# TinyMPC/TinyMPC

Measured on AMD Instinct MI355X. Metric: QP solves/sec (+ ADMM iters/sec), 64k-batch quadrotor hover, higher is better.
Workload: dtype f64; 1 GPU; quadrotor_hovering (nx=12, nu=4, N=10), 65536 identical instances per GPU, closed-loop MPC steps from a cold start (BASELINE configs[1]); batch_per_gpu=65536, total_batch=65536, parallelism=batch-sharded x1, mpc_steps_per_launch=8, stats_exchange=none (one rank), launcher=plain process

## Files before the change

### tinympc_amd/csrc/admm_kernel.hip.h

```cpp
#pragma once
#include <hip/hip_runtime.h>
#include <stdint.h>

namespace tinympc_amd {

enum : int {
    VEC_CB = 0,
    VEC_CF = 1,
    VEC_QR = 2,
    VEC_SMASK = 3,
    VEC_NIM = 4,
    VEC_SOCFLAG = 5,
    VEC_CONE_BASE = 6,
    VEC_CONE_MU = 7,
    VEC_RHO = 8,
    VEC_LINFLAG = 9,
    VEC_TLINFLAG = 10,
    VEC_COUNT = 16,
};
struct LaneTab {
    int cols, lw;
    constexpr int MB() const { return 0; }
    constexpr int MF1() const { return cols * lw; }
    constexpr int MF2() const { return 2 * cols * lw; }
// ... 40 lines not shown
    double* dbg_pd;
    uint2* accum;
    int* iter_log;
    double* u0_log;
    double rho, tol_pri, tol_dua;
    int batch, max_iter, check_termination;
    int steps;
    const double* traj;
    const int* traj_offsets;
    int traj_points, traj_step0;
    int reset_duals;
    const double* het_tabs;
    double *lslack, *ldual, *tlslack, *tldual;
    int n_lin, n_tlin;
    int cold, store_mask;
    const int* index;
    const int* count;
    int iter_base;
    int* next_index;
    int* next_count;
    double *arho, *aK, *aP, *aC1, *aC2;
    const double* atab;
    double arho_min, arho_max;
    int aclip;
    int ref_shared;
    int* work_counter;
    int reverse;
    const int* perm;
    int perm_count;
    double* vz_stream;
    int pf_mask, pf_shards, pf_static;
    unsigned* pf_counter;
    unsigned pf_base[8];
};

#define DPP_FMA(acc, src, m, lane, bank) "v_fmac_f64_dpp %[" acc "], %[" src "], %[" m "] row_newbcast:" lane " row_mask:0xf bank_mask:" bank "\n\t"
#define DPP_REP1(S) S(0, 0)
#define DPP_REP2(S) DPP_REP1(S) S(1, 1)
#define DPP_REP3(S) DPP_REP2(S) S(2, 0)
#define DPP_REP4(S) DPP_REP3(S) S(3, 1)
#define DPP_REP5(S) DPP_REP4(S) S(4, 0)
#define DPP_REP6(S) DPP_REP5(S) S(5, 1)
#define DPP_REP7(S) DPP_REP6(S) S(6, 0)
#define DPP_REP8(S) DPP_REP7(S) S(7, 1)
#define DPP_REP9(S) DPP_REP8(S) S(8, 0)
#define DPP_REP10(S) DPP_REP9(S) S(9, 1)
#define DPP_REP11(S) DPP_REP10(S) S(10, 0)
#define DPP_REP12(S) DPP_REP11(S) S(11, 1)
#define DPP_REP13(S) DPP_REP12(S) S(12, 0)
#define DPP_REP14(S) DPP_REP13(S) S(13, 1)
#define DPP_REP15(S) DPP_REP14(S) S(14, 0)
#define DPP_REP16(S) DPP_REP15(S) S(15, 1)
#define DPP_REP_(K, S) DPP_REP##K(S)
#define DPP_REP(K, S) DPP_REP_(K, S)
#define DPP_ROW_M(k, p) , [m##k] "v"(m[k])
#define DPP_ROW_A(k, p) , [a##k] "v"(ma[k])
#define DPP_ROW_B(k, p) , [b##k] "v"(mb_[k])
#define RING2_COL(k, p) DPP_FMA("a" #p, "src", "m" #k, "%[c0]+" #k, "0xf")
#define RING1_COL(k, p) DPP_FMA("a0", "src", "m" #k, "%[c0]+" #k, "0xf")
#define RING_CASE(K)                                                                                                                     \
    if constexpr (NCOL == K)                                                                                                             \
        asm("s_nop 1\n\t" DPP_REP(K, RING2_COL) : [a0] "+&v"(a0), [a1] "+&v"(a1) : [src] "v"(src), [c0] "i"(COL0) DPP_REP(K, DPP_ROW_M));
#define RING1_CASE(K)                                                                                                                    \
    if constexpr (NCOL == K)                                                                                                             \
        asm("s_nop 1\n\t" DPP_REP(K, RING1_COL) : [a0] "+&v"(a0) : [src] "v"(src), [c0] "i"(COL0) DPP_REP(K, DPP_ROW_M));

// ... 183 lines not shown
    if constexpr (fused_shape(NA, NB)) {
        double vm;
        asm("v_add_f64 %[tt], %[xi], %[g]\n\t"
            "v_max_f64 %[vm], %[lo], %[tt]\n\t"
            DPP_REP(TINYMPC_FUSED_NX, HFWD_COL_A_LO)
            "v_min_f64 %[vn], %[hi], %[vm]\n\t"
            DPP_REP(TINYMPC_FUSED_NX, HFWD_COL_A_HI)
            "v_mov_b64 %[xn], %[t]\n\t"
            "v_add_f64 %[gnew], %[tt], -%[vn]\n\t"
            DPP_REP(TINYMPC_FUSED_NU, HFWD_COL_B_LO)
            "s_nop 0\n\t"
            DPP_REP(TINYMPC_FUSED_NU, HFWD_COL_B_HI)
            : [tt] "=&v"(tt), [vm] "=&v"(vm), [vn] "=&v"(vn), [xn] "=&v"(xn), [t] "+&v"(t), [gnew] "=&v"(gnew)
            : [xi] "v"(xi), [g] "v"(g), [lo] "v"(lo), [hi] "v"(hi), FUSED_ROW_OPERANDS);
    }
#endif
}

__device__ __forceinline__ double vmax64(double a, double b) {
    double r;
    asm("v_max_f64 %0, %1, %2" : "=v"(r) : "v"(a), "v"(b));
    return r;
}
__device__ __forceinline__ double vmin64(double a, double b) {
    double r;
    asm("v_min_f64 %0, %1, %2" : "=v"(r) : "v"(a), "v"(b));
    return r;
}
__device__ __forceinline__ double pinned_sub64(double a, double b) {
    double r = a - b;
    asm volatile("" : "+v"(r));
    return r;
}
__device__ __forceinline__ double vclamp64(double lo, double hi, double t) {
    double r;
    asm("v_max_f64 %0, %1, %2\n\tv_min_f64 %0, %3, %0" : "=&v"(r) : "v"(lo), "v"(t), "v"(hi));
    return r;
}

__device__ __forceinline__ double vmax_abs64(double a, double b) {
    double r;
    asm("v_max_f64 %0, %1, |%2|" : "=v"(r) : "v"(a), "v"(b));
    return r;
}
template <bool OPAQUE>
__device__ __forceinline__ double resid_max(double a, double b) {
    if constexpr (OPAQUE) return vmax_abs64(a, b);
    else return fmax(a, fabs(b));
}

#ifndef TINYMPC_PRIM_STORE
#define TINYMPC_PRIM_STORE 1
#endif
#ifndef TINYMPC_REF_LOAD
#define TINYMPC_REF_LOAD 1
#endif
#ifndef TINYMPC_FULL_LINE_STORES
#define TINYMPC_FULL_LINE_STORES 2
#endif
__device__ __forceinline__ double load_ref(const double* p) {
#if TINYMPC_REF_LOAD == 1
    return __builtin_nontemporal_load(p);
#else
    return *p;
#endif
}
// ... 92 lines not shown
#pragma clang fp contract(off)
    for (int c = S0 + t; c < n; c += LPI_) {
        const int at = (inst * n + c) * csl + R0;
        const double* tk = tab + c * tab_stride;
        double z[NF], t0[NF];
#pragma unroll
        for (int r = 0; r < NF; ++r) { z[r] = pv[at + r]; t0[r] = z[r]; }
        for (int k = 0; k < nk; ++k) {
            double cv = 0.0;
#pragma unroll
            for (int r = 0; r < NF; ++r) { const double pr = tk[k * LW_ + R0 + r] * z[r]; cv = cv + pr; }
            const double bk = tk[KMAX_ * LW_ + k * LW_ + R0];
            if (cv > bk) {
                const double dist = (cv - bk) / tk[2 * KMAX_ * LW_ + k * LW_ + R0];
#pragma unroll
                for (int r = 0; r < NF; ++r) { const double pr = dist * tk[k * LW_ + R0 + r]; z[r] = z[r] - pr; }
            }
        }
#pragma unroll
        for (int r = 0; r < NF; ++r) { pv[at + r] = z[r]; pg[at + r] = t0[r] - z[r]; }
    }
}

template <int NX, int NU, int N, bool SOC, bool DBG, int MODE, int LIN = 0, bool HET = false, int KMAX = LIN_KMAX, bool ADAPT = false, bool UB = false, bool HALF = false,
          bool PF = false>
__global__ __launch_bounds__(64)
__attribute__((amdgpu_waves_per_eu(LIN != 0 ? solve_kernel_lin_waves(NX, NU, N, SOC, LIN, KMAX, UB) : solve_kernel_waves_per_simd(NX + NU, N, SOC, false, ADAPT),
                                   LIN != 0 ? solve_kernel_lin_waves(NX, NU, N, SOC, LIN, KMAX, UB) : solve_kernel_waves_per_simd(NX + NU, N, SOC, false, ADAPT))))
void admm_solve_kernel(const SolveArgs P) {
    constexpr bool LS = (LIN & 1) != 0, LT = (LIN & 2) != 0;
    constexpr int NZ = NX + NU;
    static_assert(NZ <= 16, "one instance per 16-lane DPP row");
    constexpr bool FUSED = MODE == 2 && LIN == 0 && fused_shape(NX, NU);
    static_assert(!HALF || (NZ <= 8 && FUSED && !SOC && !DBG && !HET && !ADAPT), "half rows: nx+nu <= 8, the plain box kernel on its fused step blocks");
    static_assert(!PF || (MODE == 2 && !SOC && !DBG && LIN == 0 && !HET && !ADAPT), "prefetch form: the plain box kernel");
    constexpr int RL = HALF ? 8 : 16;
    constexpr int IPW = 64 / RL;
    constexpr int RECD = N * NZ;
    constexpr int PF_PIECES = (IPW * RECD * 8 + 1023) / 1024;
    constexpr int PF_ARR = PF_PIECES * 128;
    constexpr unsigned long long RMASK = HALF ? 0xFFull : 0xFFFFull;
    const int lane = threadIdx.x & 63;
    const int j = lane & (RL - 1);
    const int grp = lane / RL;
    const bool is_state = j < NX;
    const bool is_input = (j >= NX) && (j < NZ);

    __shared__ double sPt[NX * 16];
    __shared__ double sLo[UB ? 1 : N * 16];
    __shared__ double sHi[UB ? 1 : N * 16];
    __shared__ double sLin[LS ? 3 * KMAX * 16 : 1];
    __shared__ double sTLin[LT ? 3 * N * KMAX * 16 : 1];
#ifndef TINYMPC_SOC_PD
#define TINYMPC_SOC_PD 2
#endif
    constexpr int SPD = TINYMPC_SOC_PD, SPR = SPD + 1;
    constexpr int CS = SOC ? ((NZ + 1) | 1) : 1;
    constexpr int SLOT_D = 3 * CS;
    constexpr int PL_GC = CS, PL_VC = 2 * CS;
    __shared__ double sC[SOC ? (4 * N + 1) * SLOT_D : 1];
    __shared__ double sP[ADAPT ? 4 * NX * NX : 1];
    constexpr int AKC = NX > NU ? NX : NU;
    constexpr bool HA = HET && ADAPT;
    __shared__ double sTab[(ADAPT && !HET) ? 3 * 16 * AKC : 1];
    __shared__ double sDl[ADAPT ? 4 * ADAPT_LOG : 1];
    if constexpr (ADAPT && !HET)
        for (int e = lane; e < 3 * 16 * AKC; e += 64) {
            const int t = e / (16 * AKC), r = e % (16 * AKC);
            sTab[e] = P.atab[t * 256 + (r % AKC) * 16 + r / AKC];
        }
    if constexpr (LS) for (int e = lane; e < 3 * KMAX * 16; e += 64) sLin[e] = P.tab[TAB_BOUNDS + 2 * N * 16 + e];
    if constexpr (LT) for (int e = lane; e < 3 * N * KMAX * 16; e += 64) sTLin[e] = P.tab[TAB_BOUNDS + 2 * N * 16 + 3 * KMAX * 16 + e];
    for (int e = lane; e < NX * 16; e += 64) sPt[e] = P.tab[TAB_PT + e];
    for (int e = lane; e < N * 16; e += 64) {
        if constexpr (!UB) {
            sLo[e] = P.tab[TAB_BOUNDS + e];
            sHi[e] = P.tab[TAB_BOUNDS + N * 16 + e];
        }
    }
    double mb[NZ], mf1[NX], mf2[NU];
#pragma unroll
    for (int k = 0; k < NZ; ++k) mb[k] = P.tab[TAB_MB + k * 16 + j];
#pragma unroll
    for (int k = 0; k < NX; ++k) mf1[k] = P.tab[TAB_MF1 + k * 16 + j];
#pragma unroll
    for (int k = 0; k < NU; ++k) mf2[k] = P.tab[TAB_MF2 + (NX + k) * 16 + j];
    double cb = P.tab[TAB_VEC + VEC_CB * 16 + j];
    double cf = P.tab[TAB_VEC + VEC_CF * 16 + j];
    double qr = P.tab[TAB_VEC + VEC_QR * 16 + j];
    const double smask = P.tab[TAB_VEC + VEC_SMASK * 16 + j];
    const double nim = P.tab[TAB_VEC + VEC_NIM * 16 + j];
    bool soc_lane = false, proj_lane = false;
    int cone_base = -1, cone_c = 0;
    double socmask = 0.0;
    if constexpr (SOC) {
        socmask = P.tab[TAB_VEC + VEC_SOCFLAG * 16 + j];
        soc_lane = socmask != 0.0;
        cone_base = (int)P.tab[TAB_VEC + VEC_CONE_BASE * 16 + j];
// ... 17 lines not shown
            int t = p * 16 + j;
            item_at[p] = 4 * N * SLOT_D; item_mu[p] = 1.0f;
            if (heads && p * 16 < soc_items_of(heads, NX, N)) soc_passes = p + 1;
            for (unsigned m = heads; m; m &= m - 1) {
                const int hb = __builtin_ctz(m);
                const int cnt = hb < NX ? N : N - 1;
                if (t >= 0 && t < cnt) {
                    item_at[p] = (grp * N + t + (hb < NX ? 0 : 1)) * SLOT_D + hb;
                    item_mu[p] = (float)P.tab[TAB_VEC + VEC_CONE_MU * 16 + hb];
                    t = -1;
                } else if (t >= 0) t -= cnt;
            }
            item_rmu[p] = 1.0f / item_mu[p];
            const unsigned mb_ = __float_as_uint(item_mu[p]);
            const bool p2 = (mb_ & 0x807FFFFFu) == 0u && (mb_ >> 23) >= 127u - 60u && (mb_ >> 23) <= 127u + 60u;
            if (__builtin_amdgcn_ballot_w64(!p2) != 0ull) mu_pow2 = false;
        }
    }
    bool lin_lane = false, tlin_lane = false;
    if constexpr (LS) lin_lane = P.tab[TAB_VEC + VEC_LINFLAG * 16 + j] != 0.0;
    if constexpr (LT) tlin_lane = P.tab[TAB_VEC + VEC_TLINFLAG * 16 + j] != 0.0;
    constexpr bool LPL = solve_kernel_lin_planes(NX, NU, N, SOC, LIN, KMAX, UB);
    constexpr bool LSP = LS && LPL, LTP = LT && LPL, LSR = LS && !LPL, LTR = LT && !LPL;
    constexpr int CSL = LPL ? ((NZ + 1) | 1) : 1;
    __shared__ double sLV[LSP ? 4 * N * CSL : 1], sLG[LSP ? 4 * N * CSL : 1];
    __shared__ double sTV[LTP ? 4 * N * CSL : 1], sTG[LTP ? 4 * N * CSL : 1];
    double ones[(LSR || LTR) ? 16 : 1];
#pragma unroll
    for (int k = 0; k < ((LSR || LTR) ? 16 : 1); ++k) ones[k] = 1.0;
    bool lin_x_on = false, lin_u_on = false, tlin_x_on = false, tlin_u_on = false;
    if constexpr (LS) { lin_x_on = P.tab[TAB_VEC + VEC_LINFLAG * 16] != 0.0; lin_u_on = P.tab[TAB_VEC + VEC_LINFLAG * 16 + NX] != 0.0; }
    if constexpr (LT) { tlin_x_on = P.tab[TAB_VEC + VEC_TLINFLAG * 16] != 0.0; tlin_u_on = P.tab[TAB_VEC + VEC_TLINFLAG * 16 + NX] != 0.0; }
    double rho = P.rho;
    __builtin_amdgcn_fence(__ATOMIC_RELEASE, "wavefront");
    __builtin_amdgcn_wave_barrier();

    const double lo_u = P.tab[TAB_BOUNDS + (N > 1 ? 16 : 0) + j], hi_u = P.tab[TAB_BOUNDS + N * 16 + (N > 1 ? 16 : 0) + j];
    const double lo_u0 = P.tab[TAB_BOUNDS + j], hi_u0 = P.tab[TAB_BOUNDS + N * 16 + j];
    const int ninst = PF ? P.batch : (P.index ? *P.count : (P.perm ? P.perm_count : P.batch));
    const int ntiles = (ninst + IPW - 1) / IPW;
    const bool resumed = !PF && P.index != nullptr;
    const bool has_traj = !PF && P.traj != nullptr;
    extern __shared__ __attribute__((aligned(16))) double sPF[];
    typedef const __attribute__((address_space(1))) void* pf_gptr;
    typedef __attribute__((address_space(3))) void* pf_lptr;
    constexpr int PF_S0 = 128, PF_S1 = PF_S0 + PF_ARR, PF_S2 = PF_S1 + PF_ARR, PF_S3 = PF_S2 + PF_ARR;
    auto pf_issue = [&](const int t) {
        const int tl = P.reverse ? ntiles - 1 - t : t;
        __builtin_amdgcn_global_load_lds((pf_gptr)(P.x0 + ((size_t)tl * (IPW * NX) + (size_t)lane * 2)), (pf_lptr)sPF, 16, 0, 0);
        const size_t t0 = (size_t)tl * (IPW * RECD) + (size_t)lane * 2;
        auto arr = [&](const double* p, const int at) {
#pragma unroll
            for (int q = 0; q < PF_PIECES; ++q) __builtin_amdgcn_global_load_lds((pf_gptr)(p + t0 + q * 128), (pf_lptr)(sPF + at + q * 128), 16, 0, 0);
        };
        if (!P.cold) { arr(P.slack, PF_S0); arr(P.dual, PF_S1); arr(P.slack_prev, PF_S2); }
        if (P.pf_mask & 8) arr(P.ref, P.cold ? PF_S0 : PF_S3);
    };
    unsigned pf_ticket = 0u;
    const int pf_shard = PF ? (int)(blockIdx.x % (unsigned)(P.pf_shards > 0 ? P.pf_shards : 1)) : 0;
    typedef __attribute__((address_space(1))) unsigned* pf_ctr_t;
    unsigned long long pf_ctr_bits = PF ? (unsigned long long)(P.pf_counter + 16 * pf_shard) : 0ull;
    if constexpr (PF) asm volatile("" : "+v"(pf_ctr_bits));
    const pf_ctr_t pf_ctr = (pf_ctr_t)pf_ctr_bits;
    auto pf_draw = [&]() { return lane == 0 ? __hip_atomic_fetch_add(pf_ctr, 1u, __ATOMIC_RELAXED, __HIP_MEMORY_SCOPE_AGENT) : 0u; };
    const unsigned pf_base = PF ? P.pf_base[pf_shard] : 0u;
    int pf_next = 0, pf_i = 0;
// ... 135 lines not shown
                    VP[s] = warm ? pfVP[s] : 0.0;
                    QX[s] = pfQXs[s];
                    X[s] = 0.0;
                    if (s == N - 1) ref_last = pf_rl;
                    continue;
                }
                const double r = valid ? (P.ref_shared ? P.ref[off - (size_t)b * (N * NZ)] : load_ref(P.ref + off)) : 0.0;
                VN[s] = warm ? P.slack[off] : 0.0;
                G[s] = warm ? P.dual[off] : 0.0;
                VP[s] = warm ? P.slack_prev[off] : 0.0;
                QX[s] = -(r * qr);
                X[s] = 0.0;
                if (s == N - 1) ref_last = r;
                if constexpr (SOC) {
                    double vc0 = (warm && soc_lane) ? (resumed ? P.cslack : P.prim)[off] : 0.0;
                    const double gc0 = (warm && soc_lane) ? P.cdual[off] : 0.0;
                    if (s == 0 && is_state && soc_lane && !resumed) vc0 = x0v_in;
                    sC[cw + s * SLOT_D] = vc0 - gc0;
                    sC[cw + s * SLOT_D + PL_GC] = gc0;
                    sC[cw + s * SLOT_D + PL_VC] = vc0;
                }
                if constexpr (LS) {
                    const double vl0 = (warm && lin_lane) ? (resumed ? P.lslack : P.prim)[off] : 0.0;
                    const double gl0 = (warm && lin_lane) ? P.ldual[off] : 0.0;
                    if constexpr (LSP) { sLV[cl + s * CSL] = vl0; sLG[cl + s * CSL] = gl0; } else { VL[s] = vl0; GL[s] = gl0; }
                }
                if constexpr (LT) {
                    const double vt0 = (warm && tlin_lane) ? (resumed ? P.tlslack : P.prim)[off] : 0.0;
                    const double gt0 = (warm && tlin_lane) ? P.tldual[off] : 0.0;
                    if constexpr (LTP) { sTV[cl + s * CSL] = vt0; sTG[cl + s * CSL] = gt0; } else { VT[s] = vt0; GT[s] = gt0; }
                }
                if constexpr (DBG) { Qd[s] = 0.0; Pd[s] = 0.0; Dd[s] = 0.0; }
            }
            double x0v = x0v_in;
            auto terminal_term = [&]() {
                double pt[NX];
#pragma unroll
                for (int k = 0; k < NX; ++k)
                    pt[k] = ADAPT ? sP[grp * NX * NX + k + NX * (is_state ? j : 0)] : (HET ? het[TAB_PT + k * 16 + j] : sPt[k * 16 + j]);
                double xp = 0.0;
                if constexpr (HALF) ring1_half<0, NX>(xp, ref_last, pt);
                else xp = ring_sum<MODE, 0, NX>(0.0, ref_last, pt);
                qx_last_plain = QX[N - 1];
                QX[N - 1] = is_state ? -xp : QX[N - 1];
            };
            int ndl = 0;
            auto flush_c = [&](int n) {
                __builtin_amdgcn_fence(__ATOMIC_RELEASE, "wavefront");
                __builtin_amdgcn_wave_barrier();
                if (P.aC2 && is_state) {
                    double* c2 = P.aC2 + (size_t)b * (NX * NX) + NX * j;
                    double v[NX], d[NX];
#pragma unroll
                    for (int k = 0; k < NX; ++k) { v[k] = c2[k]; d[k] = P.atab[(HA ? (size_t)b * ATAB_DOUBLES : (size_t)0) + ATAB_DC2 + k * 16 + j]; }
                    for (int i = 0; i < n; ++i) {
                        const double dl = sDl[grp * ADAPT_LOG + i];
#pragma unroll
                        for (int k = 0; k < NX; ++k) v[k] = taylor_step(v[k], dl, d[k]);
                    }
#pragma unroll
                    for (int k = 0; k < NX; ++k) c2[k] = v[k];
                }
                if (P.aC1 && j < NU) {
                    double* c1 = P.aC1 + (size_t)b * (NU * NU) + NU * j;
                    double v[NU], d[NU];
#pragma unroll
// ... 95 lines not shown
                            if constexpr (LT) ql = fma(-rho, tlin_w(N - 1), ql);
                            Qd[N - 1] = is_state ? ql : t;
                            Pd[N - 1] = t;
                        }
                    }
                    double pcur = qhi;
                    if constexpr (HALF) {
                        double tmpv = VN[N - 2] - G[N - 2];
#pragma unroll
                        for (int i = N - 2; i >= 0; --i) {
                            double qlo, res, dnp, tmpn;
                            constexpr int dummy = 0;
                            const int in = i > 0 ? i - 1 : dummy;
                            fused_backward_step_half<NX, NU>(qlo, res, dnp, tmpn, tmpv, VN[in], G[in], QX[i], rho, smask, cb, nim, cf, pcur, qhi, mb, mb + NX);
                            if (i + 1 <= N - 2) Dn[i + 1] = dnp;
                            tmpv = tmpn;
                            pcur = res;
                            qhi = qlo;
                        }
                        Dn[0] = fma(pcur, nim, cf);
                    }
#pragma unroll
                    for (int i = N - 2; i >= 0 && !HALF; --i) {
                        if constexpr (SOC) {
                            if (i >= SPD) wr[(i - SPD) % SPR] = sC[cw + (i - SPD) * SLOT_D];
                        }
                        if constexpr (LSP) { if (i >= SPD) { lvr[(i - SPD) % SPR] = sLV[cl + (i - SPD) * CSL]; lgr[(i - SPD) % SPR] = sLG[cl + (i - SPD) * CSL]; } }
                        if constexpr (LTP) { if (i >= SPD) { tvr[(i - SPD) % SPR] = sTV[cl + (i - SPD) * CSL]; tgr[(i - SPD) % SPR] = sTG[cl + (i - SPD) * CSL]; } }
                        if constexpr (SOC || LPL) __builtin_amdgcn_sched_barrier(0);
                        if constexpr (FUSED) {
                            double qlo, res;
                            if constexpr (SOC) fused_backward_step_soc<NX, NU>(qlo, res, VN[i], G[i], QX[i], wr[i % SPR], rho, smask, cb, pcur, qhi, mb, mb + NX);
                            else fused_backward_step<NX, NU>(qlo, res, VN[i], G[i], QX[i], rho, smask, cb, pcur, qhi, mb, mb + NX);
                            pcur = res;
                            Dn[i] = fma(res, nim, cf);
                            if constexpr (DBG) { Qd[i] = qlo; Pd[i] = res; Dd[i + 1] = res; }
                            qhi = qlo;
                            continue;
                        }
                        double qlo = fma(-rho, VN[i] - G[i], QX[i]);
                        if constexpr (SOC) qlo = fma(-rho, wr[i % SPR], qlo);
                        if constexpr (LS) qlo = fma(-rho, lin_w(i), qlo);
                        if constexpr (LT) qlo = fma(-rho, tlin_w(i), qlo);
                        const double res = ring_sum2<MODE, NX, NU>(fma(qlo, smask, cb), pcur, mb, qhi, mb + NX);
                        pcur = res;
                        Dn[i] = fma(res, nim, cf);
                        if constexpr (DBG) { Qd[i] = qlo; Pd[i] = res; Dd[i + 1] = res; }
                        qhi = qlo;
                    }
                    constexpr bool LAZY_RES = N <= 12;
                    constexpr bool TIGHT = FUSED && !HALF && LAZY_RES && !SOC && NX % 4 == 0;
                    double pmax = 0.0, dmax = 0.0;
                    auto slot_update = [&](const int s, const double lo, const double hi, const double gcv, const double glv, const double gtv) {
                        const double xi = X[s];
                        const double t = xi + G[s];
                        const double vn = TIGHT ? vclamp64(lo, hi, t) : vmin64(hi, vmax64(lo, t));
                        if constexpr (!LAZY_RES) {
                            pmax = resid_max<true>(pmax, xi - vn);
                            dmax = resid_max<true>(dmax, VP[s] - vn);
                        }
                        G[s] = t - vn;
                        VN[s] = vn;
                        if constexpr (SOC) {
                            sC[cw + s * SLOT_D] = fma(xi, socmask, gcv);
                        }
                        if constexpr (LSP) sLV[cl + s * CSL] = (lin_lane && (is_state || s >= 1)) ? (xi + glv) : 0.0;
                        if constexpr (LTP) sTV[cl + s * CSL] = (tlin_lane && (is_state || s >= 1)) ? (xi + gtv) : 0.0;
                        if constexpr (LSR || LTR) {
                            auto halfspaces = [&](double z, const double* tabk, const int nk) {
                                for (int k = 0; k < nk; ++k) {
                                    const double a = tabk[k * 16 + j];
                                    const double bk = tabk[KMAX * 16 + k * 16 + j];
                                    const double nn = tabk[2 * KMAX * 16 + k * 16 + j];
                                    const double prod = a * z;
                                    double cs = 0.0, ci = 0.0;
                                    ring1<0, NX>(cs, prod, ones);
                                    ring1<NX, NU>(ci, prod, ones);
                                    const double cv = is_state ? cs : ci;
                                    if (cv > bk) {
#pragma clang fp contract(off)
                                        const double pr = ((cv - bk) / nn) * a;
                                        z = z - pr;
                                    }
                                }
// ... 66 lines not shown
                                tt_d = tt; vn_d = vn;
                            } else G[i] = tt - vn;
                            VN[i] = vn;
                            if constexpr (SOC) sC[cw + i * SLOT_D] = fma(xi, socmask, gr[i % SPR]);
                            lo_c = lo_n; hi_c = hi_n;
                            continue;
                        }
                        const double t = ring_sum<MODE, 0, NX>(Dn[i], X[i], mf1);
                        X[i + 1] = ring_short<MODE, NX, NU>(t, t, mf2);
                        slot_update(i, lo_c, hi_c, gr[SOC ? i % SPR : 0], glr[LSP ? i % SPR : 0], gtr[LTP ? i % SPR : 0]);
                        lo_c = lo_n; hi_c = hi_n;
                    }
                    if constexpr (TIGHT && N >= 2) G[N - 2] = tt_d - vn_d;
                    (void)tt_d; (void)vn_d;
                    slot_update(N - 1, lo_c, hi_c, gr[SOC ? (N - 1) % SPR : 0], glr[LSP ? (N - 1) % SPR : 0], gtr[LTP ? (N - 1) % SPR : 0]);
                    if constexpr (LPL) {
                        __builtin_amdgcn_fence(__ATOMIC_RELEASE, "wavefront");
                        __builtin_amdgcn_wave_barrier();
                        if constexpr (LSP) {
                            if (lin_x_on) project_halfspace_columns<NX, KMAX, 16, 16>(j, grp, N, CSL, 0, 0, sLV, sLG, sLin, 0, P.n_lin);
                            if (lin_u_on) project_halfspace_columns<NU, KMAX, 16, 16>(j, grp, N, CSL, NX, 1, sLV, sLG, sLin, 0, P.n_lin);
                        }
                        if constexpr (LTP) {
                            if (tlin_x_on) project_halfspace_columns<NX, KMAX, 16, 16>(j, grp, N, CSL, 0, 0, sTV, sTG, sTLin, 3 * KMAX * 16, P.n_tlin);
                            if (tlin_u_on) project_halfspace_columns<NU, KMAX, 16, 16>(j, grp, N, CSL, NX, 1, sTV, sTG, sTLin, 3 * KMAX * 16, P.n_tlin);
                        }
                        __builtin_amdgcn_fence(__ATOMIC_RELEASE, "wavefront");
                        __builtin_amdgcn_wave_barrier();
                    }
                    bool conv = false;
                    auto termination = [&]() {
                        if (countdown > 0 && --countdown == 0) {
                            countdown = P.check_termination;
                            checked = 1;
                            constexpr int PS0 = N >= 2 ? 1 : 0, PS1 = N - 1;
                            auto lost = [&](const int s) {
                                return (int)(fabs(X[s] - VN[s]) >= P.tol_pri) | (int)(fabs(VP[s] - VN[s]) * rho >= P.tol_dua);
                            };
                            const bool maybe = ((int)!(rho > 0.0) | (int)!(lost(PS0) | lost(PS1))) != 0;
                            unsigned long long fold = __ballot(maybe);
                            fold &= fold >> 1; fold &= fold >> 2; fold &= fold >> 4;
                            if constexpr (!HALF) fold &= fold >> 8;
                            const bool any_row = (fold & (HALF ? 0x0101010101010101ull : 0x0001000100010001ull)) != 0ull;
                            const bool last_test = (P.max_iter - 1 - it) < P.check_termination;
                            if (last_test || any_row) {
                                if constexpr (LAZY_RES) {
#pragma unroll
                                    for (int s = 0; s < N; ++s) {
                                        pmax = resid_max<false>(pmax, X[s] - VN[s]);
                                        dmax = resid_max<false>(dmax, VP[s] - VN[s]);
                                    }
                                }
                                rp = pmax;
                                rd = dmax * rho;
                                const bool ok = (rp < P.tol_pri) && (rd < P.tol_dua);
                                const unsigned long long bal = __ballot(ok);
                                conv = ((bal >> (grp * RL)) & RMASK) == RMASK;
                            }
                        }
                    };
                    if constexpr (SOC) {
                        __builtin_amdgcn_fence(__ATOMIC_RELEASE, "wavefront");
                        __builtin_amdgcn_wave_barrier();
                        double n0 = sC[item_at[0]], n1 = sC[item_at[0] + 1], n2 = sC[item_at[0] + 2];
#pragma unroll
                        for (int d = 1; d <= SPR && d <= N; ++d) wr[(N - d) % SPR] = sC[cw + (N - d) * SLOT_D];
                        termination();
                        bool any_exact = false;
#pragma unroll
                        for (int p = 0; p < SOC_PASSES; ++p) {
                            if (p > 0 && p >= soc_passes) break;
                            const int at = item_at[p];
                            if (p > 0) { n0 = sC[at]; n1 = sC[at + 1]; n2 = sC[at + 2]; }
                            const double s0 = n0, s1 = n1, s2 = n2;
                            if (soc_all_inside(s0, s1, s2, item_mu[p])) {
                                sC[at + PL_VC] = s0; sC[at + PL_VC + 1] = s1; sC[at + PL_VC + 2] = s2;
                                if (!gcz[p]) {
                                    sC[at + PL_GC] = 0.0; sC[at + PL_GC + 1] = 0.0; sC[at + PL_GC + 2] = 0.0;
                                    gcz[p] = true;
                                }
                            } else {
                                double r0, r1, r2;
                                soc_project3(s0, s1, s2, item_mu[p], item_rmu[p], mu_pow2, r0, r1, r2);
                                const double g0 = s0 - r0, g1 = s1 - r1, g2 = s2 - r2;
                                sC[at + PL_VC] = r0; sC[at + PL_VC + 1] = r1; sC[at + PL_VC + 2] = r2;
                                sC[at + PL_GC] = g0; sC[at + PL_GC + 1] = g1; sC[at + PL_GC + 2] = g2;
                                sC[at] = r0 - g0; sC[at + 1] = r1 - g1; sC[at + 2] = r2 - g2;
                                gcz[p] = false;
                                any_exact = true;
                            }
                        }
                        if (it == iter0 && !proj_lane) {
#pragma unroll
                            for (int s = 0; s < N; ++s) sC[cw + s * SLOT_D + PL_GC] = 0.0;
                        }
                        __builtin_amdgcn_fence(__ATOMIC_RELEASE, "wavefront");
                        __builtin_amdgcn_wave_barrier();
                        if (any_exact) {
#pragma unroll
                            for (int d = 1; d <= SPR && d <= N; ++d) wr[(N - d) % SPR] = sC[cw + (N - d) * SLOT_D];
                        }
                    }
                    iter += 1;
                    if constexpr (ADAPT) {
                        if (it > 0 && it % 5 == 0) {
                            double at[NX];
#pragma unroll
                            for (int k = 0; k < NX; ++k) at[k] = HA ? atab_i[ATAB_AT + k * 16 + j] : sTab[j * AKC + k];
                            double pri_res = 0.0, ax_max = 0.0, z_max = 0.0, dual_res = 0.0, px_max = 0.0, aty_max = 0.0, q_max = 0.0;
                            double pxq_max = 0.0;
#pragma unroll
                            for (int i = 0; i < N - 1; ++i) {
                                const double axs = ring_sum<MODE, 0, NX>(0.0, X[i], mf1);
                                const double dyn = ring_short<MODE, NX, NU>(axs, is_input ? X[i + 1] : 0.0, mf2) - X[i + 1];
                                const double a = is_state ? dyn : X[i + 1];
                                const double zz = VN[i + 1];
                                const bool on = is_state || is_input;
                                pri_res = fmax(pri_res, on ? fabs(a - zz) : 0.0);
                                ax_max = fmax(ax_max, on ? fabs(a) : 0.0);
                                z_max = fmax(z_max, on ? fabs(zz) : 0.0);
                                const double init = is_state ? (i >= 1 ? -G[i] : 0.0) : G[i + 1];
                                const double aty = ring_sum<MODE, 0, NX>(init, G[i + 1], at);
                                const double xs = is_state ? X[i] : X[i + 1];
                                const double px = qr * xs;
                                dual_res = fmax(dual_res, on ? fabs((px + px) + aty) : 0.0);
                                pxq_max = fmax(pxq_max, on ? fabs(px) : 0.0);
                                aty_max = fmax(aty_max, on ? fabs(aty) : 0.0);
                            }
                            {
                                double prow[NX];
#pragma unroll
                                for (int k = 0; k < NX; ++k) prow[k] = sP[grp * NX * NX + (is_state ? j : 0) + NX * k];
                                const double pxl = ring_sum<MODE, 0, NX>(0.0, X[N - 1], prow);
                                const double ql = qr * X[N - 1];
                                const double atyl = -G[N - 1];
                                dual_res = fmax(dual_res, is_state ? fabs((pxl + ql) + atyl) : 0.0);
// ... 6 lines not shown
                            const double pri_norm = fmax(ax_max, z_max);
                            const double dual_norm = fmax(fmax(px_max, aty_max), q_max);
                            const double eps = 1e-10;
                            const double normalized_pri = pri_res / (pri_norm + eps);
                            const double normalized_dual = dual_res / (dual_norm + eps);
                            const double ratio = normalized_pri / (normalized_dual + eps);
                            double new_rho = rho * sqrt(ratio);
                            if (P.aclip) new_rho = fmin(fmax(new_rho, P.arho_min), P.arho_max);
                            const double delta = new_rho - rho;
                            if (is_state) {
#pragma unroll
                                for (int k = 0; k < NU; ++k) mb[NX + k] = -taylor_step(-mb[NX + k], delta, (HA ? atab_i[ATAB_DK + k * 16 + j] : sTab[(16 + j) * AKC + k]));
#pragma unroll
                                for (int k = 0; k < NX; ++k) {
                                    const int e = grp * NX * NX + k + NX * j;
                                    sP[e] = taylor_step(sP[e], delta, (HA ? atab_i[ATAB_DP + k * 16 + j] : sTab[(32 + j) * AKC + k]));
                                }
                            } else if (is_input) {
#pragma unroll
                                for (int k = 0; k < NX; ++k) mf1[k] = -taylor_step(-mf1[k], delta, (HA ? atab_i[ATAB_DK + k * 16 + j] : sTab[(16 + j) * AKC + k]));
                            }
                            if (P.aC1 || P.aC2) {
                                if (j == 0) sDl[grp * ADAPT_LOG + ndl] = delta;
                                if (++ndl == ADAPT_LOG) { flush_c(ndl); ndl = 0; }
                            }
                            rho = new_rho;
                            __builtin_amdgcn_fence(__ATOMIC_RELEASE, "wavefront");
                            __builtin_amdgcn_wave_barrier();
                            QX[N - 1] = qx_last_plain;
                            terminal_term();
                        }
                    }
                    if constexpr (!SOC) termination();
                    if (conv) { solved = 1; break; }
#pragma unroll
                    for (int s = 0; s < N; ++s) VP[s] = VN[s];
                    vp_touched = true;
                }
                acc_iter += (unsigned)(iter - iter0);
                acc_solved += (unsigned)solved;
                if (P.iter_log && j == 0) P.iter_log[(size_t)step * P.batch + b] = solved ? iter : -iter;
                if (P.u0_log && is_input) P.u0_log[((size_t)step * P.batch + b) * NU + (j - NX)] = X[1];
                if (nsteps > 1) {
                    x0v = is_state ? X[1] : 0.0;
                }
            }

            constexpr bool FLS = TINYMPC_FULL_LINE_STORES != 0 && (PF || TINYMPC_FULL_LINE_STORES == 2) && !SOC && LIN == 0 && !DBG;
            if (FLS && (P.store_mask & 32) == 0) {
                if constexpr (FLS) {
                    const size_t seg = (size_t)b * (N * NZ) + j;
                    const bool in_row = j < NZ;
#pragma unroll
                    for (int s = 0; s < N; ++s) {
                        const size_t off = seg + s * NZ;
                        const double xs = is_input ? (s + 1 < N ? X[s + 1 < N ? s + 1 : s] : 0.0) : X[s];
                        const double vs = is_input ? (s + 1 < N ? VN[s + 1 < N ? s + 1 : s] : 0.0) : VN[s];
                        const double gs = is_input ? (s + 1 < N ? G[s + 1 < N ? s + 1 : s] : 0.0) : G[s];
                        const double ps = is_input ? (s + 1 < N ? VP[s + 1 < N ? s + 1 : s] : 0.0) : VP[s];
                        if (in_row) {
                            if (P.store_mask & 1) {
                                if (acc_iter > 0) { if constexpr (PF) P.prim[off] = xs; else store_primal(P.prim + off, xs); }
                                else if (s == 0 && is_state) P.prim[off] = xs;
                            }
                            if (P.store_mask & 2) P.slack[off] = vs;
                            if (P.store_mask & 4) P.dual[off] = gs;
                            if ((P.store_mask & 8) && vp_touched) P.slack_prev[off] = ps;
                        }
                    }
                }
            } else
#pragma unroll
            for (int s = 0; s < N; ++s) {
                const bool valid = is_state || (is_input && s >= 1);
                const size_t off = lbase + s * NZ;
                if (valid) {
                    if (((P.store_mask & 1) || ((P.store_mask & 32) && s <= 1)) && (acc_iter > 0 || (s == 0 && is_state))) {
                        if constexpr (SOC || LIN != 0) P.prim[off] = X[s];
                        else store_primal(P.prim + off, X[s]);
                    }
                    if (P.store_mask & 2) P.slack[off] = VN[s];
                    if (P.store_mask & 4) P.dual[off] = G[s];
                    if ((P.store_mask & 8) && vp_touched) P.slack_prev[off] = VP[s];
                    if constexpr (SOC) {
                        if (soc_lane && (P.store_mask & 16)) {
                            P.cslack[off] = sC[cw + s * SLOT_D + ((proj_lane || iter <= iter_first) ? PL_VC : 0)];
                            P.cdual[off] = sC[cw + s * SLOT_D + PL_GC];
                        }
                    }
                    if constexpr (LSP) { if (lin_lane && (P.store_mask & 16)) { P.lslack[off] = sLV[cl + s * CSL]; P.ldual[off] = sLG[cl + s * CSL]; } }
                    if constexpr (LTP) { if (tlin_lane && (P.store_mask & 16)) { P.tlslack[off] = sTV[cl + s * CSL]; P.tldual[off] = sTG[cl + s * CSL]; } }
                    if constexpr (LSR) { if (lin_lane && (P.store_mask & 16)) { P.lslack[off] = VL[s]; P.ldual[off] = GL[s]; } }
                    if constexpr (LTR) { if (tlin_lane && (P.store_mask & 16)) { P.tlslack[off] = VT[s]; P.tldual[off] = GT[s]; } }
                    if constexpr (DBG) {
                        if (P.dbg_qr && acc_iter > 0) {
                            P.dbg_qr[off] = Qd[s];
                            P.dbg_pd[off] = is_state ? Pd[s] : Dd[s];
                        }
                    }
                }
            }
            if constexpr (ADAPT) {
                if (ndl > 0) flush_c(ndl);
                if (j == 0) P.arho[b] = rho;
                if (is_state) {
#pragma unroll
                    for (int k = 0; k < NU; ++k) P.aK[(size_t)b * (NU * NX) + k + NU * j] = -mb[NX + k];
#pragma unroll
                    for (int k = 0; k < NX; ++k) P.aP[(size_t)b * (NX * NX) + k + NX * j] = sP[grp * NX * NX + k + NX * j];
                }
            }
            if (P.x0_next && acc_iter > 0 && is_state) P.x0_next[(size_t)b * NX + j] = X[1];
            const double ps = grp_maxw<RL>(is_state ? rp : 0.0), pi = grp_maxw<RL>(is_input ? rp : 0.0);
            const double ds = grp_maxw<RL>(is_state ? rd : 0.0), di = grp_maxw<RL>(is_input ? rd : 0.0);
            if (P.next_index) {
                const bool open = j == 0 && !solved;
// ... 31 lines not shown
```

### tinympc_amd/csrc/batch_dispatch.hip

```cpp
#define TINYMPC_GENERAL_KERNEL_IMPL
#include "batch_impl.hpp"
#include "batch_dispatch.hpp"

#include <algorithm>
#include <cstdarg>
#include <cstdio>
#include <cstring>
#include <limits>
#include <string>

namespace tinympc_amd {

#include "_gen/registry.inc"
const int g_nkernels = (int)(sizeof(g_kernels) / sizeof(g_kernels[0]));
const KernelEntry* const* const g_kernel_list = g_kernels;

static const int g_ntiles = (int)(sizeof(g_tiles) / sizeof(g_tiles[0]));
const TileEntry* find_tile(int nx, int nu, int N) {
    for (int i = 0; i < g_ntiles; ++i)
        if (g_tiles[i]->nx == nx && g_tiles[i]->nu == nu && g_tiles[i]->N == N) return g_tiles[i];
    return nullptr;
}
static int variant_tile_r(const TinyBatch* b) {
    int r = b->tile ? b->tile->R : 1;
    for (int i = 0; i < g_ntiles; ++i)
        if (g_tiles[i]->nx == b->nx && g_tiles[i]->nu == b->nu && g_tiles[i]->N == b->N) r = g_tiles[i]->R;
    return r;
}
static int soc_families(const TinyBatch* b) {
    return ((b->set.en_input_soc && !b->Acu.empty()) ? 1 : 0) | ((b->set.en_state_soc && !b->Acx.empty()) ? 2 : 0);
}
static int lin_families(const TinyBatch* b) {
    return ((b->set.en_state_linear || b->set.en_input_linear) ? 1 : 0) | ((b->set.en_tv_state_linear || b->set.en_tv_input_linear) ? 2 : 0);
}
static int budget_variant_tile_r(const TinyBatch* b, int socm, int lv, int km, bool ub) {
// ... 85 lines not shown
    b->ttab_gen = b->tab_gen;
    build_tile_tables(b);
    return upload_growing(b, &b->d_ttab, &b->ttab_doubles, b->h_ttab);
}

static int launch_waves(const TinyBatch* b, int count, int ipw) {
    const int tiles = (count + ipw - 1) / ipw;
    return b->grid_waves_per_cu > 0 ? (int)std::min<long>(tiles, (long)b->num_cus * b->grid_waves_per_cu) : tiles;
}
static int timing_begin(TinyBatch* b, bool* timed) {
    *timed = b->timing_left > 0 && b->timing_n < (int)b->ev_start.size();
    if (*timed) HIP_TRY(b, hipEventRecord(b->ev_start[b->timing_n], b->stream));
    return TINY_OK;
}
static int timing_end(TinyBatch* b, bool timed) {
    if (!timed) return TINY_OK;
    HIP_TRY(b, hipEventRecord(b->ev_stop[b->timing_n], b->stream));
    b->timing_n++; b->timing_left--;
    return TINY_OK;
}

static int bind_halfspace_slacks(TinyBatch* b, int lv, SolveArgs& a) {
    if (lv & 1) { if (int rc = ensure_kpi(b, &b->d_lslack)) return rc; if (int rc = ensure_kpi(b, &b->d_ldual)) return rc; }
    if (lv & 2) { if (int rc = ensure_kpi(b, &b->d_tlslack)) return rc; if (int rc = ensure_kpi(b, &b->d_tldual)) return rc; }
    a.lslack = b->d_lslack; a.ldual = b->d_ldual; a.tlslack = b->d_tlslack; a.tldual = b->d_tldual;
    a.n_lin = std::max(b->set.en_state_linear ? b->nsl : 0, b->set.en_input_linear ? b->nil : 0);
    a.n_tlin = std::max(b->set.en_tv_state_linear ? b->ntsl : 0, b->set.en_tv_input_linear ? b->ntil : 0);
    return TINY_OK;
}
static int bind_common_args(TinyBatch* b, SolveArgs& a) {
    a.x0 = b->d_x0; a.ref = b->d_ref; a.prim = b->d_prim; a.slack = b->d_slack; a.dual = b->d_dual; a.slack_prev = b->d_slack_prev;
    a.cslack = b->d_cslack; a.cdual = b->d_cdual; a.status = b->d_status; a.resid = b->d_resid; a.accum = b->d_accum;
    a.rho = b->cache.rho; a.tol_pri = b->set.abs_pri_tol; a.tol_dua = b->set.abs_dua_tol;
    a.batch = b->batch; a.max_iter = b->set.max_iter; a.check_termination = b->set.check_termination;
    a.steps = b->steps_per_launch > 1 ? b->steps_per_launch : 1;
    a.x0_next = (b->advance_x0 || a.steps > 1) ? b->d_x0 : nullptr;
    a.store_mask = b->one_shot == 2 ? 1 : (b->one_shot == 1 ? 3 : 31);
    a.traj = b->d_traj; a.traj_offsets = b->d_traj_offsets; a.traj_points = b->traj_points; a.traj_step0 = (int)b->traj_step;
    a.reset_duals = b->reset_duals ? 1 : 0;
    if (a.steps > 1 && b->step_log) {
        if (int rc = ensure_step_logs(b, a.steps)) return rc;
        a.iter_log = b->d_iter_log; a.u0_log = b->d_u0_log;
    }
    return TINY_OK;
}

struct TileLaunch {
    const TileEntry* te = nullptr;
    SolveKernel k = nullptr;
    hipFunction_t jit_fn = nullptr;
    int W = 1, R = 1, soc = 0, lin = 0, kmax = LIN_KMAX, ext = 0, lm = 0;
    bool ub = false, dyn = false;
    int ipw = 4, grid = 0, resident = 0;
    bool honours_index = false;
    const void* key() const { return jit_fn ? reinterpret_cast<const void*>(jit_fn) : reinterpret_cast<const void*>(k); }
};
enum TileVerdict {
    TILE_GO,
    TILE_VARIANT_FAILED,
    TILE_EXT_REFUSED,
    TILE_SHAPE_DROPPED,
    TILE_NO_ENTRY,
    TILE_HET_LAYOUT,
};

static bool jit_dynamic_slots(const TinyBatch* b, int ipw) {
// ... 788 lines not shown
```

Before: 2.871 billion QP solves/s.

## Slim fused box kernel: spill VP slots to LDS and precompute dual threshold

For the fused plain box kernel (SLIM), the interior previous-slack slots VP move from registers to per-lane LDS, with only the two probe slots kept in registers. This lowers VGPR pressure and could raise occupancy. The termination probe now compares against a host-precomputed dual threshold (tol_dua/rho, nudged to the exact float boundary) using split ballots, so the multiply leaves the check. The backward pass is rescheduled with pinned FMAs, and the per-iteration iter counter and flags are now computed once after the loop. The risks are extra LDS traffic on every iteration and changed instruction scheduling.

After: 2.841 billion QP solves/s. 1.1% lower.

```diff
diff --git a/tinympc_amd/csrc/admm_kernel.hip.h b/tinympc_amd/csrc/admm_kernel.hip.h
--- a/tinympc_amd/csrc/admm_kernel.hip.h
+++ b/tinympc_amd/csrc/admm_kernel.hip.h
@@ -96,6 +96,7 @@
     int pf_mask, pf_shards, pf_static;
     unsigned* pf_counter;
     unsigned pf_base[8];
+    double thr_dua;
 };
 
 #define DPP_FMA(acc, src, m, lane, bank) "v_fmac_f64_dpp %[" acc "], %[" src "], %[" m "] row_newbcast:" lane " row_mask:0xf bank_mask:" bank "\n\t"
@@ -345,6 +346,11 @@
     asm volatile("" : "+v"(r));
     return r;
 }
+__device__ __forceinline__ double pinned_fma64(double a, double b, double c) {
+    double r = fma(a, b, c);
+    asm volatile("" : "+v"(r));
+    return r;
+}
 __device__ __forceinline__ double vclamp64(double lo, double hi, double t) {
     double r;
     asm("v_max_f64 %0, %1, %2\n\tv_min_f64 %0, %3, %0" : "=&v"(r) : "v"(lo), "v"(t), "v"(hi));
@@ -503,6 +509,12 @@
     constexpr int NZ = NX + NU;
     static_assert(NZ <= 16, "one instance per 16-lane DPP row");
     constexpr bool FUSED = MODE == 2 && LIN == 0 && fused_shape(NX, NU);
+    constexpr bool SLIM = FUSED && !HALF && N <= 12 && !SOC && NX % 4 == 0 && !DBG;
+#ifndef TINYMPC_VP_LDS
+#define TINYMPC_VP_LDS 1
+#endif
+    constexpr bool VPL = SLIM && !PF && N > 2 && TINYMPC_VP_LDS != 0;
+    constexpr int PS0 = N >= 2 ? 1 : 0, PS1 = N - 1;
     static_assert(!HALF || (NZ <= 8 && FUSED && !SOC && !DBG && !HET && !ADAPT), "half rows: nx+nu <= 8, the plain box kernel on its fused step blocks");
     static_assert(!PF || (MODE == 2 && !SOC && !DBG && LIN == 0 && !HET && !ADAPT), "prefetch form: the plain box kernel");
     constexpr int RL = HALF ? 8 : 16;
@@ -535,6 +547,21 @@
     constexpr bool HA = HET && ADAPT;
     __shared__ double sTab[(ADAPT && !HET) ? 3 * 16 * AKC : 1];
     __shared__ double sDl[ADAPT ? 4 * ADAPT_LOG : 1];
+    double* sVP = nullptr;
+    if constexpr (VPL) {
+        __shared__ double sVP_[(N - 2) * 64];
+        sVP = sVP_ + lane;
+    }
+    (void)sVP;
+    auto vp_row = [](const int s) { return (s == 0 ? 0 : s - 1) * 64; };
+    auto vp_get = [&](const double* vp, const int s) {
+        if constexpr (VPL) { if (s != PS0 && s != PS1) return sVP[vp_row(s)]; }
+        return vp[s];
+    };
+    auto vp_set = [&](double* vp, const int s, const double v) {
+        if constexpr (VPL) { if (s != PS0 && s != PS1) { sVP[vp_row(s)] = v; return; } }
+        vp[s] = v;
+    };
     if constexpr (ADAPT && !HET)
         for (int e = lane; e < 3 * 16 * AKC; e += 64) {
             const int t = e / (16 * AKC), r = e % (16 * AKC);
@@ -618,6 +645,7 @@
     if constexpr (LS) { lin_x_on = P.tab[TAB_VEC + VEC_LINFLAG * 16] != 0.0; lin_u_on = P.tab[TAB_VEC + VEC_LINFLAG * 16 + NX] != 0.0; }
     if constexpr (LT) { tlin_x_on = P.tab[TAB_VEC + VEC_TLINFLAG * 16] != 0.0; tlin_u_on = P.tab[TAB_VEC + VEC_TLINFLAG * 16 + NX] != 0.0; }
     double rho = P.rho;
+    if constexpr (SLIM && !HET && !ADAPT) asm("" : "+v"(rho));
     __builtin_amdgcn_fence(__ATOMIC_RELEASE, "wavefront");
     __builtin_amdgcn_wave_barrier();
 
@@ -819,6 +847,10 @@
                 }
                 if constexpr (DBG) { Qd[s] = 0.0; Pd[s] = 0.0; Dd[s] = 0.0; }
             }
+            if constexpr (VPL) {
+#pragma unroll
+                for (int s = 0; s < N; ++s) vp_set(VP, s, VP[s]);
+            }
             double x0v = x0v_in;
             auto terminal_term = [&]() {
                 double pt[NX];
@@ -980,6 +1012,14 @@
                             double qlo, res;
                             if constexpr (SOC) fused_backward_step_soc<NX, NU>(qlo, res, VN[i], G[i], QX[i], wr[i % SPR], rho, smask, cb, pcur, qhi, mb, mb + NX);
                             else fused_backward_step<NX, NU>(qlo, res, VN[i], G[i], QX[i], rho, smask, cb, pcur, qhi, mb, mb + NX);
+                            if constexpr (SLIM) {
+                                __builtin_amdgcn_sched_barrier(0);
+                                if (i < N - 2) Dn[i + 1] = pinned_fma64(pcur, nim, cf);
+                                pcur = res;
+                                if (i == 0) Dn[0] = fma(res, nim, cf);
+                                qhi = qlo;
+                                continue;
+                            }
                             pcur = res;
                             Dn[i] = fma(res, nim, cf);
                             if constexpr (DBG) { Qd[i] = qlo; Pd[i] = res; Dd[i + 1] = res; }
@@ -998,6 +1038,7 @@
                     }
                     constexpr bool LAZY_RES = N <= 12;
                     constexpr bool TIGHT = FUSED && !HALF && LAZY_RES && !SOC && NX % 4 == 0;
+                    static_assert(SLIM == (TIGHT && !DBG), "SLIM: the TIGHT forms without the debug records");
                     double pmax = 0.0, dmax = 0.0;
                     auto slot_update = [&](const int s, const double lo, const double hi, const double gcv, const double glv, const double gtv) {
                         const double xi = X[s];
@@ -1130,19 +1171,40 @@
                     auto termination = [&]() {
                         if (countdown > 0 && --countdown == 0) {
                             countdown = P.check_termination;
-                            checked = 1;
-                            constexpr int PS0 = N >= 2 ? 1 : 0, PS1 = N - 1;
+                            if constexpr (!SLIM) checked = 1;
                             auto lost = [&](const int s) {
                                 return (int)(fabs(X[s] - VN[s]) >= P.tol_pri) | (int)(fabs(VP[s] - VN[s]) * rho >= P.tol_dua);
                             };
-                            const bool maybe = ((int)!(rho > 0.0) | (int)!(lost(PS0) | lost(PS1))) != 0;
-                            unsigned long long fold = __ballot(maybe);
+                            unsigned long long fold;
+                            if constexpr (SLIM) {
+                                auto vote = [](const bool c) { return (unsigned long long)__builtin_amdgcn_ballot_w64(c); };
+                                auto kept = [&](const int s) {
+                                    if constexpr (!HET && !ADAPT) return vote(!(fabs(X[s] - VN[s]) >= P.tol_pri)) & vote(!(fabs(VP[s] - VN[s]) >= P.thr_dua));
+                                    else return vote(!(fabs(X[s] - VN[s]) >= P.tol_pri)) & vote(!(fabs(VP[s] - VN[s]) * rho >= P.tol_dua));
+                                };
+                                fold = kept(PS0) & kept(PS1);
+                                if constexpr (HET || ADAPT) fold |= vote(!(rho > 0.0));
+                            } else {
+                                const bool maybe = ((int)!(rho > 0.0) | (int)!(lost(PS0) | lost(PS1))) != 0;
+                                fold = __ballot(maybe);
+                            }
                             fold &= fold >> 1; fold &= fold >> 2; fold &= fold >> 4;
                             if constexpr (!HALF) fold &= fold >> 8;
-                            const bool any_row = (fold & (HALF ? 0x0101010101010101ull : 0x0001000100010001ull)) != 0ull;
+                            bool any_row = (fold & (HALF ? 0x0101010101010101ull : 0x0001000100010001ull)) != 0ull;
+                            if constexpr (SLIM && !HET && !ADAPT) any_row |= !(P.rho > 0.0);
                             const bool last_test = (P.max_iter - 1 - it) < P.check_termination;
                             if (last_test || any_row) {
-                                if constexpr (LAZY_RES) {
+                                if constexpr (VPL) {
+                                    double vp[N];
+#pragma unroll
+                                    for (int s = 0; s < N; ++s) vp[s] = vp_get(VP, s);
+                                    __builtin_amdgcn_sched_barrier(0);
+#pragma unroll
+                                    for (int s = N - 1; s >= 0; --s) {
+                                        pmax = resid_max<false>(pmax, X[s] - VN[s]);
+                                        dmax = resid_max<false>(dmax, vp[s] - VN[s]);
+                                    }
+                                } else if constexpr (LAZY_RES) {
 #pragma unroll
                                     for (int s = 0; s < N; ++s) {
                                         pmax = resid_max<false>(pmax, X[s] - VN[s]);
@@ -1152,8 +1214,11 @@
                                 rp = pmax;
                                 rd = dmax * rho;
                                 const bool ok = (rp < P.tol_pri) && (rd < P.tol_dua);
-                                const unsigned long long bal = __ballot(ok);
+                                unsigned long long bal;
+                                if constexpr (SLIM) bal = (unsigned long long)__builtin_amdgcn_ballot_w64(rp < P.tol_pri) & (unsigned long long)__builtin_amdgcn_ballot_w64(rd < P.tol_dua);
+                                else bal = __ballot(ok);
                                 conv = ((bal >> (grp * RL)) & RMASK) == RMASK;
+                                if constexpr (SLIM) { if (conv) { iter = it + 1; solved = 1; } }
                             }
                         }
                     };
@@ -1199,7 +1264,7 @@
                             for (int d = 1; d <= SPR && d <= N; ++d) wr[(N - d) % SPR] = sC[cw + (N - d) * SLOT_D];
                         }
                     }
-                    iter += 1;
+                    if constexpr (!SLIM) iter += 1;
                     if constexpr (ADAPT) {
                         if (it > 0 && it % 5 == 0) {
                             double at[NX];
@@ -1272,10 +1337,16 @@
                         }
                     }
                     if constexpr (!SOC) termination();
-                    if (conv) { solved = 1; break; }
-#pragma unroll
-                    for (int s = 0; s < N; ++s) VP[s] = VN[s];
-                    vp_touched = true;
+                    if constexpr (SLIM) { if (conv) break; }
+                    else if (conv) { solved = 1; break; }
+#pragma unroll
+                    for (int s = 0; s < N; ++s) vp_set(VP, s, VN[s]);
+                    if constexpr (!SLIM) vp_touched = true;
+                }
+                if constexpr (SLIM) {
+                    if (!solved) iter = P.max_iter > iter0 ? P.max_iter : iter0;
+                    if (iter - iter0 > solved) vp_touched = true;
+                    if (P.check_termination > 0 && (long long)P.max_iter - iter0 >= P.check_termination) checked = 1;
                 }
                 acc_iter += (unsigned)(iter - iter0);
                 acc_solved += (unsigned)solved;
@@ -1297,7 +1368,7 @@
                         const double xs = is_input ? (s + 1 < N ? X[s + 1 < N ? s + 1 : s] : 0.0) : X[s];
                         const double vs = is_input ? (s + 1 < N ? VN[s + 1 < N ? s + 1 : s] : 0.0) : VN[s];
                         const double gs = is_input ? (s + 1 < N ? G[s + 1 < N ? s + 1 : s] : 0.0) : G[s];
-                        const double ps = is_input ? (s + 1 < N ? VP[s + 1 < N ? s + 1 : s] : 0.0) : VP[s];
+                        const double ps = is_input ? (s + 1 < N ? vp_get(VP, s + 1 < N ? s + 1 : s) : 0.0) : vp_get(VP, s);
                         if (in_row) {
                             if (P.store_mask & 1) {
                                 if (acc_iter > 0) { if constexpr (PF) P.prim[off] = xs; else store_primal(P.prim + off, xs); }
@@ -1321,7 +1392,7 @@
                     }
                     if (P.store_mask & 2) P.slack[off] = VN[s];
                     if (P.store_mask & 4) P.dual[off] = G[s];
-                    if ((P.store_mask & 8) && vp_touched) P.slack_prev[off] = VP[s];
+                    if ((P.store_mask & 8) && vp_touched) P.slack_prev[off] = vp_get(VP, s);
                     if constexpr (SOC) {
                         if (soc_lane && (P.store_mask & 16)) {
                             P.cslack[off] = sC[cw + s * SLOT_D + ((proj_lane || iter <= iter_first) ? PL_VC : 0)];
diff --git a/tinympc_amd/csrc/batch_dispatch.hip b/tinympc_amd/csrc/batch_dispatch.hip
--- a/tinympc_amd/csrc/batch_dispatch.hip
+++ b/tinympc_amd/csrc/batch_dispatch.hip
@@ -1,6 +1,7 @@
 #define TINYMPC_GENERAL_KERNEL_IMPL
 #include "batch_impl.hpp"
 #include "batch_dispatch.hpp"
+#include "probe_threshold.hpp"
 
 #include <algorithm>
 #include <cstdarg>
@@ -152,6 +153,7 @@
     a.x0 = b->d_x0; a.ref = b->d_ref; a.prim = b->d_prim; a.slack = b->d_slack; a.dual = b->d_dual; a.slack_prev = b->d_slack_prev;
     a.cslack = b->d_cslack; a.cdual = b->d_cdual; a.status = b->d_status; a.resid = b->d_resid; a.accum = b->d_accum;
     a.rho = b->cache.rho; a.tol_pri = b->set.abs_pri_tol; a.tol_dua = b->set.abs_dua_tol;
+    a.thr_dua = probe_dual_threshold(a.tol_dua, a.rho);
     a.batch = b->batch; a.max_iter = b->set.max_iter; a.check_termination = b->set.check_termination;
     a.steps = b->steps_per_launch > 1 ? b->steps_per_launch : 1;
     a.x0_next = (b->advance_x0 || a.steps > 1) ? b->d_x0 : nullptr;
diff --git a/tinympc_amd/csrc/probe_threshold.hpp b/tinympc_amd/csrc/probe_threshold.hpp
--- /dev/null
+++ b/tinympc_amd/csrc/probe_threshold.hpp
@@ -0,0 +1,31 @@
+#pragma once
+#include <cmath>
+#include <limits>
+
+namespace tinympc_amd {
+
+enum : int { PROBE_THRESHOLD_MAX_STEPS = 8 };
+
+inline double probe_dual_threshold(const double tol_dua, const double rho) {
+    const double nan = std::numeric_limits<double>::quiet_NaN(), inf = std::numeric_limits<double>::infinity();
+    if (!(rho > 0.0) || !std::isfinite(rho) || !std::isfinite(tol_dua)) return nan;
+    if (tol_dua <= 0.0) return 0.0;
+    auto reaches = [&](const double x) { volatile double p = x * rho; return p >= tol_dua; };
+    double thr = tol_dua / rho;
+    int steps = 0;
+    if (reaches(thr)) {
+        for (;;) {
+            const double below = std::nextafter(thr, -inf);
+            if (!(below >= 0.0) || !reaches(below)) return thr;
+            if (++steps > PROBE_THRESHOLD_MAX_STEPS) return nan;
+            thr = below;
+        }
+    }
+    while (!reaches(thr)) {
+        if (++steps > PROBE_THRESHOLD_MAX_STEPS) return nan;
+        thr = std::nextafter(thr, inf);
+    }
+    return thr;
+}
+
+}
```
